# Onetism/LightFieldMicroscopy_PC-bzip2

Hardware: NVIDIA B200
Metric: compress+decompress round-trip GB/s (raw uint16) (higher is better)
Workload: dtype u16

## Files before the change

lightfieldmicroscopy_pc-bzip2_b200/csrc/bz_bwt.cu:

```cuda
#include "lfm_radix.cuh"
#include <cstdlib>

namespace lfm {

enum { S_SA0 = 0, S_SA1, S_ISA, S_G0, S_G1, S_R0, S_R1, S_V0, S_V1, S_U0, S_U1, S_COUNT };

extern __shared__ __align__(16) uint8_t bwt_smem[];

template <int NT>
__global__ void __launch_bounds__(NT, NT == 1024 ? 1 : 4)
k_bwt(const uint8_t* __restrict__ txt_all, uint32_t cap, EncJob* __restrict__ jobs, uint32_t njobs,
      uint8_t* __restrict__ bwt_all, uint32_t* __restrict__ scratch_all, int text_in_smem, int prefix_forced)
{
	constexpr int BWT_NT = NT;
	uint32_t* wcnt = reinterpret_cast<uint32_t*>(bwt_smem);
	uint32_t* base = reinterpret_cast<uint32_t*>(bwt_smem + (NT / 32) * BWT_WS * 4);
	uint32_t* run  = base + 256;
	uint32_t* red  = run + 256;
	uint32_t* misc = red + 64;
	uint8_t*  stext = reinterpret_cast<uint8_t*>(misc + 16);

	uint32_t* scr = scratch_all + (size_t)blockIdx.x * S_COUNT * cap;
	const uint32_t tid = threadIdx.x;

	for (uint32_t job = blockIdx.x; job < njobs; job += gridDim.x) {
		const uint32_t n = jobs[job].n;
		const uint8_t* gtext = txt_all + (size_t)job * cap;
		uint8_t* bwt = bwt_all + (size_t)job * cap;
		if (n == 0) { if (tid == 0) { jobs[job].orig_ptr = 0; jobs[job].periodic = 0; } continue; }

		const uint8_t* text;
		if (text_in_smem) {
			for (uint32_t i = tid * 4; i < n; i += BWT_NT * 4) {
				uint32_t wv = *reinterpret_cast<const uint32_t*>(gtext + i);
				*reinterpret_cast<uint32_t*>(stext + i) = wv;
			}
			__syncthreads();
			if (tid < 8) stext[n + tid] = stext[tid % n];
			text = stext;
		} else {
			text = gtext;
		}
		__syncthreads();
		digit_starts<NT>(n, base, wcnt, red, [&](uint32_t e) { return (uint32_t)text[e]; });
		if (tid < 256) {
			const uint32_t c = (tid == 255 ? n : base[tid + 1]) - base[tid];
			const uint32_t bal = __ballot_sync(0xffffffffu, c != 0);
			if ((tid & 31) == 0) jobs[job].in_use[tid >> 5] = bal;
		}

		const int prefix = prefix_forced ? prefix_forced : (n <= 49152u ? 6 : 8);
		uint32_t* src = nullptr; uint32_t* dst = scr + (size_t)S_SA0 * cap;
		for (int p = prefix - 1; p >= 0; p--) {
			if (tid < 256) run[tid] = base[tid];
			__syncthreads();
			const uint32_t* s = src; uint32_t* d = dst;
			radix_scatter<BWT_R, uint32_t, NT>(n, run, wcnt,
				[&](uint32_t e) { return s ? s[e] : e; },
				[&](uint32_t idx) { return (uint32_t)text[idx + p]; },
				[&](uint32_t pos, uint32_t idx) { d[pos] = idx; });
			src = dst;
			dst = (dst == scr + (size_t)S_SA0 * cap) ? scr + (size_t)S_SA1 * cap : scr + (size_t)S_SA0 * cap;
		}
		uint32_t* sa = src;
		uint32_t* isa = scr + (size_t)S_ISA * cap;

		uint32_t* G[2] = { scr + (size_t)S_G0 * cap, scr + (size_t)S_G1 * cap };
		uint32_t* Rk[2] = { scr + (size_t)S_R0 * cap, scr + (size_t)S_R1 * cap };
		uint32_t* V[2] = { scr + (size_t)S_V0 * cap, scr + (size_t)S_V1 * cap };
		uint32_t* U[2] = { scr + (size_t)S_U0 * cap, scr + (size_t)S_U1 * cap };
		const uint64_t pmask = prefix >= 8 ? ~0ull : ((1ull << (8 * prefix)) - 1ull);
		uint32_t m = split_groups<NT>(n, red,
			[&](uint32_t j) -> uint64_t {
				const uint32_t idx = sa[j], sh = (idx & 3u) * 8u;
				const uint32_t* tw = reinterpret_cast<const uint32_t*>(text + (idx & ~3u));
				const uint32_t w0 = tw[0], w1 = tw[1], w2 = tw[2];
				return (((uint64_t)__funnelshift_r(w1, w2, sh) << 32) | __funnelshift_r(w0, w1, sh)) & pmask;
			},
			[&](uint32_t j) { return j; },
			[&](uint32_t j, uint32_t head, bool un, uint32_t slot) {
				uint32_t sfx = sa[j];
				isa[sfx] = head;
				if (un) { G[0][slot] = head; V[0][slot] = sfx; U[0][slot] = j; }
			});

		const int npass = n <= (1u << 8) ? 1 : n <= (1u << 16) ? 2 : 3;
		int cur = 0, ucur = 0;
		uint64_t h = (uint64_t)prefix;
		while (m > 0 && h < n) {
			uint32_t hh = (uint32_t)h;
			for (uint32_t e = tid; e < m; e += BWT_NT) {
				uint32_t i = V[cur][e] + hh; if (i >= n) i -= n;
				Rk[cur][e] = isa[i];
			}
			__syncthreads();
			for (int key = 0; key < 2; key++) {
				for (int ps = 0; ps < npass; ps++) {
					const uint32_t* kg = G[cur]; const uint32_t* kr = Rk[cur]; const uint32_t* kv = V[cur];
					uint32_t* og = G[cur ^ 1]; uint32_t* orr = Rk[cur ^ 1]; uint32_t* ov = V[cur ^ 1];
					const int sh = ps * 8;
					digit_starts<NT>(m, run, wcnt, red, [&](uint32_t e) { return ((key ? kg[e] : kr[e]) >> sh) & 255u; });
					radix_scatter<4, Trip, NT>(m, run, wcnt,
						[&](uint32_t e) { Trip t; t.g = kg[e]; t.r = kr[e]; t.v = kv[e]; return t; },
						[&](const Trip& t) { return ((key ? t.g : t.r) >> sh) & 255u; },
						[&](uint32_t pos, const Trip& t) { og[pos] = t.g; orr[pos] = t.r; ov[pos] = t.v; });
					cur ^= 1;
				}
			}
			{
				const uint32_t* kg = G[cur]; const uint32_t* kr = Rk[cur]; const uint32_t* kv = V[cur];
				const uint32_t* up = U[ucur];
				uint32_t* ng = G[cur ^ 1]; uint32_t* nv = V[cur ^ 1]; uint32_t* nu = U[ucur ^ 1];
				const uint32_t mm = m;
				m = split_groups<NT>(mm, red,
					[&](uint32_t s) -> uint64_t { return ((uint64_t)kg[s] << 32) | kr[s]; },
					[&](uint32_t s) { return up[s]; },
					[&](uint32_t s, uint32_t head, bool un, uint32_t slot) {
						uint32_t sfx = kv[s], pos = up[s];
						sa[pos] = sfx;
						isa[sfx] = head;
						if (un) { ng[slot] = head; nv[slot] = sfx; nu[slot] = pos; }
					});
				cur ^= 1; ucur ^= 1;
			}
			__syncthreads();
			h <<= 1;
		}

		for (uint32_t j = tid * 4; j < n; j += BWT_NT * 4) {
			const uint4 q = *reinterpret_cast<const uint4*>(sa + j);
			const uint32_t sv[4] = { q.x, q.y, q.z, q.w };
			uint32_t wv = 0;
			#pragma unroll
			for (int k = 0; k < 4; k++) if (j + k < n) {
				const uint32_t s = sv[k];
				wv |= (uint32_t)text[s ? s - 1 : n - 1] << (8 * k);
				if (s == 0 && m == 0) jobs[job].orig_ptr = j + k;
			}
			*reinterpret_cast<uint32_t*>(bwt + j) = wv;
		}
		if (m > 0) {
			if (tid == 0) misc[1] = 0;
			__syncthreads();
			uint32_t g0 = isa[0], c = 0;
			for (uint32_t e = tid; e < m; e += BWT_NT) c += (G[cur][e] == g0);
			if (c) atomicAdd(&misc[1], c);
			__syncthreads();
			if (tid == 0) jobs[job].orig_ptr = g0 + misc[1] - 1;
		}
		if (tid == 0) jobs[job].periodic = m > 0;
		__syncthreads();
	}
}

static size_t bwt_smem_bytes_nt(uint32_t cap, int text_in_smem, int nt)
{
	size_t fixed = (size_t)(nt / 32) * BWT_WS * 4 + (256 + 256 + 64 + 16) * 4;
	return fixed + (text_in_smem ? (size_t)cap + 16 : 0);
}
size_t bwt_smem_bytes(uint32_t cap, int text_in_smem) { return bwt_smem_bytes_nt(cap, text_in_smem, BWT_NT); }
size_t bwt_scratch_elems_per_cta(uint32_t cap) { return (size_t)S_COUNT * cap; }
int bwt_ctas_per_sm(uint32_t cap, int text_in_smem)
{
	static const int forced = getenv("LFM_B200_BWT_NT") ? atoi(getenv("LFM_B200_BWT_NT")) : 0;
	if (forced == 1024) return 1;
	return (text_in_smem && bwt_smem_bytes_nt(cap, 1, 256) + 1024 <= (size_t)227 * 1024 / 4) ? 4 : 1;
}

void launch_bwt(const uint8_t* txt, uint32_t cap, EncJob* jobs, uint32_t njobs, uint8_t* bwt, uint32_t* scratch,
                int grid, int text_in_smem, cudaStream_t st)
{
	static const int prefix = getenv("LFM_B200_BWT_PREFIX") ? std::min(8, std::max(2, atoi(getenv("LFM_B200_BWT_PREFIX")))) : 0;
	if (bwt_ctas_per_sm(cap, text_in_smem) == 4) {
		const size_t smem = bwt_smem_bytes_nt(cap, text_in_smem, 256);
		cudaFuncSetAttribute(k_bwt<256>, cudaFuncAttributeMaxDynamicSharedMemorySize, (int)smem);
		k_bwt<256><<<grid, 256, smem, st>>>(txt, cap, jobs, njobs, bwt, scratch, text_in_smem, prefix);
		return;
	}
	const size_t smem = bwt_smem_bytes_nt(cap, text_in_smem, 1024);
	cudaFuncSetAttribute(k_bwt<1024>, cudaFuncAttributeMaxDynamicSharedMemorySize, (int)smem);
	k_bwt<1024><<<grid, 1024, smem, st>>>(txt, cap, jobs, njobs, bwt, scratch, text_in_smem, prefix);
}

}
```

lightfieldmicroscopy_pc-bzip2_b200/csrc/lfm_radix.cuh:

```cuda
#pragma once
#include "lfm_device.cuh"

namespace lfm {

constexpr int BWT_NT = 1024;
constexpr int BWT_R  = 12;
constexpr int BWT_NW = BWT_NT / 32;
constexpr int BWT_WS = 257;
constexpr int SPLIT_R = 4;
#define LFM_WC(w, d) wcnt[(w) * BWT_WS + (d)]

struct Trip { uint32_t g, r, v; };

template <int R, class P, int NT = BWT_NT, class LoadFn, class DigitFn, class StoreFn>
__device__ __forceinline__ void radix_scatter(uint32_t m, uint32_t* run, uint32_t* wcnt,
                                              LoadFn load, DigitFn digit, StoreFn store)
{
	const uint32_t lane = lane_id(), w = warp_id();
	const uint32_t lt = (1u << lane) - 1u;
	constexpr uint32_t TILE = NT * R;
	uint32_t* myc = wcnt + w * BWT_WS;
	__syncthreads();
	for (uint32_t i = lane; i < BWT_WS; i += 32) myc[i] = 0;
	__syncwarp();
	for (uint32_t t0 = 0; t0 < m; t0 += TILE) {
		P pay[R]; uint32_t dl[R];
		const uint32_t eb = t0 + w * (32 * R) + lane;
		#pragma unroll
		for (int r = 0; r < R; r++) if (eb + r * 32 < m) pay[r] = load(eb + r * 32);
		#pragma unroll
		for (int r = 0; r < R; r++) dl[r] = (eb + r * 32 < m) ? digit(pay[r]) : 256u;
		constexpr int RH = R > 8 ? R / 2 : R;
		#pragma unroll
		for (int r0 = 0; r0 < R; r0 += RH) {
			uint32_t peers[RH], old[RH];
			#pragma unroll
			for (int r = 0; r < RH; r++) peers[r] = __match_any_sync(0xffffffffu, dl[r0 + r]);
			#pragma unroll
			for (int r = 0; r < RH; r++) {
				old[r] = 0;
				if ((peers[r] & lt) == 0) old[r] = atomicAdd(&myc[dl[r0 + r]], (uint32_t)__popc(peers[r]));
				__syncwarp();
			}
			#pragma unroll
			for (int r = 0; r < RH; r++) {
				const uint32_t o = __shfl_sync(0xffffffffu, old[r], __ffs(peers[r]) - 1);
				dl[r0 + r] = (dl[r0 + r] << 16) | (o + __popc(peers[r] & lt));
			}
		}
		__syncthreads();
		if constexpr (NT == 256) {
			const uint32_t d = threadIdx.x;
			uint32_t* col = wcnt + d;
			uint32_t c[8];
			#pragma unroll
			for (int i = 0; i < 8; i++) c[i] = col[i * BWT_WS];
			uint32_t acc = run[d];
			#pragma unroll
			for (int i = 0; i < 8; i++) { col[i * BWT_WS] = acc; acc += c[i]; }
			run[d] = acc;
		} else {
			static_assert(NT == 1024, "scan layouts exist for 1024 and 256 threads");
			const uint32_t d = threadIdx.x >> 2, part = threadIdx.x & 3u;
			uint32_t* col = wcnt + (part * 8) * BWT_WS + d;
			uint32_t c[8], tot = 0;
			#pragma unroll
			for (int i = 0; i < 8; i++) { c[i] = col[i * BWT_WS]; tot += c[i]; }
			uint32_t incl = tot;
			uint32_t t1 = __shfl_up_sync(0xffffffffu, incl, 1); if (part >= 1) incl += t1;
			uint32_t t2 = __shfl_up_sync(0xffffffffu, incl, 2); if (part >= 2) incl += t2;
			uint32_t acc = run[d] + incl - tot;
			#pragma unroll
			for (int i = 0; i < 8; i++) { col[i * BWT_WS] = acc; acc += c[i]; }
			__syncwarp();
			if (part == 3) run[d] = acc;
		}
		__syncthreads();
		#pragma unroll
		for (int r = 0; r < R; r++) if (eb + r * 32 < m) store(myc[dl[r] >> 16] + (dl[r] & 0xffffu), pay[r]);
		__syncwarp();
		for (uint32_t i = lane; i < BWT_WS; i += 32) myc[i] = 0;
		__syncwarp();
	}
	__syncthreads();
}

template <bool SCAN, int NT = BWT_NT, class DigitOfIndex>
__device__ __forceinline__ void digit_hist(uint32_t m, uint32_t* run, uint32_t* wcnt, uint32_t* red, DigitOfIndex dig)
{
	const uint32_t lane = lane_id(), w = warp_id();
	const uint32_t lt = (1u << lane) - 1u;
	uint32_t* myc = wcnt + w * BWT_WS;
	constexpr int U = 4;
	__syncthreads();
	for (uint32_t i = lane; i < BWT_WS; i += 32) myc[i] = 0;
	__syncwarp();
	for (uint32_t e0 = w * (32 * U); e0 < m; e0 += NT * U) {
		uint32_t d[U], peers[U];
		#pragma unroll
		for (int u = 0; u < U; u++) { const uint32_t e = e0 + u * 32 + lane; d[u] = e < m ? dig(e) : 256u; }
		#pragma unroll
		for (int u = 0; u < U; u++) peers[u] = __match_any_sync(0xffffffffu, d[u]);
		#pragma unroll
		for (int u = 0; u < U; u++) if ((peers[u] & lt) == 0) atomicAdd(&myc[d[u]], (uint32_t)__popc(peers[u]));
	}
	__syncthreads();
	if (threadIdx.x < 256) {
		uint32_t s = 0;
		#pragma unroll 8
		for (int ww = 0; ww < NT / 32; ww++) s += LFM_WC(ww, threadIdx.x);
		run[threadIdx.x] = s;
	}
	__syncthreads();
	if (SCAN) scan256_excl<NT>(run, red);
}
template <int NT = BWT_NT, class DigitOfIndex>
__device__ __forceinline__ void digit_starts(uint32_t m, uint32_t* run, uint32_t* wcnt, uint32_t* red, DigitOfIndex dig)
{
	digit_hist<true, NT>(m, run, wcnt, red, dig);
}

template <int NT = BWT_NT, class KeyFn, class PosFn, class EmitFn>
__device__ __forceinline__ uint32_t split_groups(uint32_t cnt, uint32_t* red, KeyFn key_of, PosFn pos_of, EmitFn emit)
{
	uint32_t carry_head = 0, carry_cnt = 0;
	for (uint32_t t0 = 0; t0 < cnt; t0 += NT * SPLIT_R) {
		uint32_t i0 = t0 + threadIdx.x * SPLIT_R;
		bool hd[SPLIT_R + 1]; uint32_t gh[SPLIT_R];
		{
			uint64_t ky[SPLIT_R + 2];
			#pragma unroll
			for (int r = 0; r < SPLIT_R + 2; r++) { const uint32_t j = i0 + r; ky[r] = (j >= 1 && j <= cnt) ? key_of(j - 1) : 0; }
			#pragma unroll
			for (int r = 0; r <= SPLIT_R; r++) { const uint32_t j = i0 + r; hd[r] = (j == 0 || j >= cnt) ? true : (ky[r] != ky[r + 1]); }
		}
		uint32_t local = 0;
		#pragma unroll
		for (int r = 0; r < SPLIT_R; r++) { if (i0 + r < cnt && hd[r]) local = pos_of(i0 + r); gh[r] = local; }
		uint32_t incl = block_scan_max<NT>(local, red);
		uint32_t tile_max = red[NT / 32 - 1];
		uint32_t before = __shfl_up_sync(0xffffffffu, incl, 1);
		if (lane_id() == 0) before = warp_id() ? red[warp_id() - 1] : 0;
		before = max(before, carry_head);
		uint32_t c = 0; bool un[SPLIT_R];
		#pragma unroll
		for (int r = 0; r < SPLIT_R; r++) {
			gh[r] = max(gh[r], before);
			un[r] = (i0 + r < cnt) && !(hd[r] && hd[r + 1]);
			c += un[r];
		}
		uint32_t tot; uint32_t inc = block_scan_add<NT>(c, red, &tot);
		uint32_t o = carry_cnt + inc - c;
		#pragma unroll
		for (int r = 0; r < SPLIT_R; r++) if (i0 + r < cnt) { emit(i0 + r, gh[r], un[r], o); o += un[r]; }
		carry_cnt += tot;
		carry_head = max(carry_head, tile_max);
	}
	__syncthreads();
	return carry_cnt;
}

}
```

Measured before the change: 2.399.

## Sort BWT prefix by dense byte-pair ranks with segmented counting passes

When the block has at most 2048 distinct byte pairs, the kernel builds a bitmap of the pairs present, gives each pair a dense 16-bit rank, and sorts the initial prefix by these ranks. This halves the number of LSD radix passes. Each pass is a segmented counting sort that packs two 16-bit counters into each shared word and carries the rank in the upper bits of the stored value. It adds an extra pass over the text, a rank array written into the ISA scratch space, and a larger shared-memory footprint. Optional clock64 phase instrumentation is included behind a compile flag.

Result: slower. 2.262, median of 6 (-5.7%).

```diff
diff --git a/lightfieldmicroscopy_pc-bzip2_b200/csrc/bz_bwt.cu b/lightfieldmicroscopy_pc-bzip2_b200/csrc/bz_bwt.cu
--- a/lightfieldmicroscopy_pc-bzip2_b200/csrc/bz_bwt.cu
+++ b/lightfieldmicroscopy_pc-bzip2_b200/csrc/bz_bwt.cu
@@ -2,6 +2,19 @@
 #include <cstdlib>
 
 namespace lfm {
+
+#ifdef LFM_BWT_PHASE_CLOCKS
+__device__ unsigned long long bwt_phase_cycles[5];
+#define BWT_PHASE(k) do { if (tid == 0) { const long long t1 = clock64(); atomicAdd(&bwt_phase_cycles[k], (unsigned long long)(t1 - t_ph)); t_ph = t1; } } while (0)
+#else
+#define BWT_PHASE(k) do { } while (0)
+#endif
+
+__host__ __device__ constexpr size_t bwt_cnt_bytes(int nt, bool pairs)
+{
+	return (size_t)(nt / 32) * BWT_WS * 4 + 512 * 4 > (pairs ? (size_t)(nt / 32) * SEG_NB * 2 : 0)
+	     ? (size_t)(nt / 32) * BWT_WS * 4 + 512 * 4 : (size_t)(nt / 32) * SEG_NB * 2;
+}
 
 enum { S_SA0 = 0, S_SA1, S_ISA, S_G0, S_G1, S_R0, S_R1, S_V0, S_V1, S_U0, S_U1, S_COUNT };
 
@@ -10,13 +23,13 @@
 template <int NT>
 __global__ void __launch_bounds__(NT, NT == 1024 ? 1 : 4)
 k_bwt(const uint8_t* __restrict__ txt_all, uint32_t cap, EncJob* __restrict__ jobs, uint32_t njobs,
-      uint8_t* __restrict__ bwt_all, uint32_t* __restrict__ scratch_all, int text_in_smem, int prefix_forced)
+      uint8_t* __restrict__ bwt_all, uint32_t* __restrict__ scratch_all, int text_in_smem, int prefix_forced, int pair_smem)
 {
 	constexpr int BWT_NT = NT;
 	uint32_t* wcnt = reinterpret_cast<uint32_t*>(bwt_smem);
 	uint32_t* base = reinterpret_cast<uint32_t*>(bwt_smem + (NT / 32) * BWT_WS * 4);
 	uint32_t* run  = base + 256;
-	uint32_t* red  = run + 256;
+	uint32_t* red  = reinterpret_cast<uint32_t*>(bwt_smem + bwt_cnt_bytes(NT, pair_smem));
 	uint32_t* misc = red + 64;
 	uint8_t*  stext = reinterpret_cast<uint8_t*>(misc + 16);
 
@@ -28,6 +41,9 @@
 		const uint8_t* gtext = txt_all + (size_t)job * cap;
 		uint8_t* bwt = bwt_all + (size_t)job * cap;
 		if (n == 0) { if (tid == 0) { jobs[job].orig_ptr = 0; jobs[job].periodic = 0; } continue; }
+#ifdef LFM_BWT_PHASE_CLOCKS
+		long long t_ph = clock64();
+#endif
 
 		const uint8_t* text;
 		if (text_in_smem) {
@@ -42,26 +58,72 @@
 			text = gtext;
 		}
 		__syncthreads();
-		digit_starts<NT>(n, base, wcnt, red, [&](uint32_t e) { return (uint32_t)text[e]; });
-		if (tid < 256) {
-			const uint32_t c = (tid == 255 ? n : base[tid + 1]) - base[tid];
-			const uint32_t bal = __ballot_sync(0xffffffffu, c != 0);
-			if ((tid & 31) == 0) jobs[job].in_use[tid >> 5] = bal;
-		}
-
 		const int prefix = prefix_forced ? prefix_forced : (n <= 49152u ? 6 : 8);
+		uint16_t* rho = reinterpret_cast<uint16_t*>(scr + (size_t)S_ISA * cap);
+		bool pairs = false;
+		uint32_t D = 0;
+		if (NT == 256 && pair_smem && (prefix & 1) == 0) {
+			uint32_t* bm = wcnt;
+			uint16_t* wpre = reinterpret_cast<uint16_t*>(wcnt + 2048);
+			for (uint32_t i = tid; i < 2048 / 4; i += BWT_NT) reinterpret_cast<uint4*>(bm)[i] = make_uint4(0, 0, 0, 0);
+			__syncthreads();
+			for (uint32_t i = tid; i < n; i += BWT_NT) {
+				const uint32_t key = (uint32_t)text[i] << 8 | text[i + 1], bit = 1u << (key & 31);
+				if (!(bm[key >> 5] & bit)) atomicOr(&bm[key >> 5], bit);
+			}
+			__syncthreads();
+			uint32_t c[8], cs = 0;
+			#pragma unroll
+			for (int k = 0; k < 8; k++) { c[k] = __popc(bm[8 * tid + k]); cs += c[k]; }
+			uint32_t pre = block_scan_add<NT>(cs, red, &D) - cs;
+			#pragma unroll
+			for (int k = 0; k < 8; k++) { wpre[8 * tid + k] = (uint16_t)pre; pre += c[k]; }
+			pairs = D <= (uint32_t)SEG_NB;
+			if (pairs) {
+				const uint32_t bal = __ballot_sync(0xffffffffu, cs != 0);
+				if ((tid & 31) == 0) jobs[job].in_use[tid >> 5] = bal;
+				__syncthreads();
+				for (uint32_t i = tid; i < n + 4; i += BWT_NT) {
+					const uint32_t key = (uint32_t)text[i] << 8 | text[i + 1];
+					rho[i] = (uint16_t)(wpre[key >> 5] + __popc(bm[key >> 5] & ((1u << (key & 31)) - 1u)));
+				}
+			}
+			__syncthreads();
+		}
+		if (!pairs) {
+			digit_starts<NT>(n, base, wcnt, red, [&](uint32_t e) { return (uint32_t)text[e]; });
+			if (tid < 256) {
+				const uint32_t c = (tid == 255 ? n : base[tid + 1]) - base[tid];
+				const uint32_t bal = __ballot_sync(0xffffffffu, c != 0);
+				if ((tid & 31) == 0) jobs[job].in_use[tid >> 5] = bal;
+			}
+		}
+		BWT_PHASE(0);
+
 		uint32_t* src = nullptr; uint32_t* dst = scr + (size_t)S_SA0 * cap;
-		for (int p = prefix - 1; p >= 0; p--) {
-			if (tid < 256) run[tid] = base[tid];
-			__syncthreads();
+		const int npass = pairs ? prefix / 2 : prefix;
+		const uint32_t nbits = D > 1 ? 32 - __clz(D - 1) : 0;
+		for (int p = npass - 1; p >= 0; p--) {
 			const uint32_t* s = src; uint32_t* d = dst;
-			radix_scatter<BWT_R, uint32_t, NT>(n, run, wcnt,
-				[&](uint32_t e) { return s ? s[e] : e; },
-				[&](uint32_t idx) { return (uint32_t)text[idx + p]; },
-				[&](uint32_t pos, uint32_t idx) { d[pos] = idx; });
+			if (pairs) {
+				const uint32_t off = 2 * p;
+				if constexpr (NT == 256)
+					seg_counting_pass<NT>(n, nbits, wcnt, red,
+						[&](uint32_t e) { return s ? s[e] : (uint32_t)rho[e + off] << 16 | e; },
+						[&](uint32_t v) { const uint32_t idx = v & 0xffffu; return p ? (uint32_t)rho[idx + off - 2] << 16 | idx : idx; },
+						[&](uint32_t pos, uint32_t v) { d[pos] = v; });
+			} else {
+				if (tid < 256) run[tid] = base[tid];
+				__syncthreads();
+				radix_scatter<BWT_R, uint32_t, NT>(n, run, wcnt,
+					[&](uint32_t e) { return s ? s[e] : e; },
+					[&](uint32_t idx) { return (uint32_t)text[idx + p]; },
+					[&](uint32_t pos, uint32_t idx) { d[pos] = idx; });
+			}
 			src = dst;
 			dst = (dst == scr + (size_t)S_SA0 * cap) ? scr + (size_t)S_SA1 * cap : scr + (size_t)S_SA0 * cap;
 		}
+		BWT_PHASE(1);
 		uint32_t* sa = src;
 		uint32_t* isa = scr + (size_t)S_ISA * cap;
 
@@ -83,8 +145,9 @@
 				isa[sfx] = head;
 				if (un) { G[0][slot] = head; V[0][slot] = sfx; U[0][slot] = j; }
 			});
-
-		const int npass = n <= (1u << 8) ? 1 : n <= (1u << 16) ? 2 : 3;
+		BWT_PHASE(2);
+
+		const int nrpass = n <= (1u << 8) ? 1 : n <= (1u << 16) ? 2 : 3;
 		int cur = 0, ucur = 0;
 		uint64_t h = (uint64_t)prefix;
 		while (m > 0 && h < n) {
@@ -95,7 +158,7 @@
 			}
 			__syncthreads();
 			for (int key = 0; key < 2; key++) {
-				for (int ps = 0; ps < npass; ps++) {
+				for (int ps = 0; ps < nrpass; ps++) {
 					const uint32_t* kg = G[cur]; const uint32_t* kr = Rk[cur]; const uint32_t* kv = V[cur];
 					uint32_t* og = G[cur ^ 1]; uint32_t* orr = Rk[cur ^ 1]; uint32_t* ov = V[cur ^ 1];
 					const int sh = ps * 8;
@@ -126,6 +189,7 @@
 			__syncthreads();
 			h <<= 1;
 		}
+		BWT_PHASE(3);
 
 		for (uint32_t j = tid * 4; j < n; j += BWT_NT * 4) {
 			const uint4 q = *reinterpret_cast<const uint4*>(sa + j);
@@ -150,12 +214,13 @@
 		}
 		if (tid == 0) jobs[job].periodic = m > 0;
 		__syncthreads();
+		BWT_PHASE(4);
 	}
 }
 
-static size_t bwt_smem_bytes_nt(uint32_t cap, int text_in_smem, int nt)
-{
-	size_t fixed = (size_t)(nt / 32) * BWT_WS * 4 + (256 + 256 + 64 + 16) * 4;
+static size_t bwt_smem_bytes_nt(uint32_t cap, int text_in_smem, int nt, bool pairs = false)
+{
+	size_t fixed = bwt_cnt_bytes(nt, pairs) + (64 + 16) * 4;
 	return fixed + (text_in_smem ? (size_t)cap + 16 : 0);
 }
 size_t bwt_smem_bytes(uint32_t cap, int text_in_smem) { return bwt_smem_bytes_nt(cap, text_in_smem, BWT_NT); }
@@ -171,15 +236,17 @@
                 int grid, int text_in_smem, cudaStream_t st)
 {
 	static const int prefix = getenv("LFM_B200_BWT_PREFIX") ? std::min(8, std::max(2, atoi(getenv("LFM_B200_BWT_PREFIX")))) : 0;
+	static const bool pairs_on = !(getenv("LFM_B200_BWT_PAIRS") && atoi(getenv("LFM_B200_BWT_PAIRS")) == 0);
 	if (bwt_ctas_per_sm(cap, text_in_smem) == 4) {
-		const size_t smem = bwt_smem_bytes_nt(cap, text_in_smem, 256);
+		const bool pairs = pairs_on && bwt_smem_bytes_nt(cap, 1, 256, true) + 1024 <= (size_t)227 * 1024 / 4;
+		const size_t smem = bwt_smem_bytes_nt(cap, text_in_smem, 256, pairs);
 		cudaFuncSetAttribute(k_bwt<256>, cudaFuncAttributeMaxDynamicSharedMemorySize, (int)smem);
-		k_bwt<256><<<grid, 256, smem, st>>>(txt, cap, jobs, njobs, bwt, scratch, text_in_smem, prefix);
+		k_bwt<256><<<grid, 256, smem, st>>>(txt, cap, jobs, njobs, bwt, scratch, text_in_smem, prefix, (int)pairs);
 		return;
 	}
 	const size_t smem = bwt_smem_bytes_nt(cap, text_in_smem, 1024);
 	cudaFuncSetAttribute(k_bwt<1024>, cudaFuncAttributeMaxDynamicSharedMemorySize, (int)smem);
-	k_bwt<1024><<<grid, 1024, smem, st>>>(txt, cap, jobs, njobs, bwt, scratch, text_in_smem, prefix);
-}
-
-}
+	k_bwt<1024><<<grid, 1024, smem, st>>>(txt, cap, jobs, njobs, bwt, scratch, text_in_smem, prefix, 0);
+}
+
+}
diff --git a/lightfieldmicroscopy_pc-bzip2_b200/csrc/lfm_radix.cuh b/lightfieldmicroscopy_pc-bzip2_b200/csrc/lfm_radix.cuh
--- a/lightfieldmicroscopy_pc-bzip2_b200/csrc/lfm_radix.cuh
+++ b/lightfieldmicroscopy_pc-bzip2_b200/csrc/lfm_radix.cuh
@@ -120,6 +120,105 @@
 	digit_hist<true, NT>(m, run, wcnt, red, dig);
 }
 
+constexpr int SEG_NB = 2048;
+#ifndef SEG_HIST_MATCH
+#define SEG_HIST_MATCH 1
+#endif
+#ifndef SEG_BALLOT
+#define SEG_BALLOT 0
+#endif
+#ifndef SEG_NBITS_ALL
+#define SEG_NBITS_ALL 1
+#endif
+__device__ __forceinline__ uint32_t seg_peers(uint32_t d, bool valid, uint32_t nbits)
+{
+#if SEG_BALLOT
+	uint32_t p = __ballot_sync(0xffffffffu, valid);
+	#pragma unroll
+	for (int b = 0; b < 11; b++)
+		if (SEG_NBITS_ALL || b < nbits) { const uint32_t q = __ballot_sync(0xffffffffu, (d >> b) & 1u); p &= ((d >> b) & 1u) ? q : ~q; }
+	return p;
+#else
+	return __match_any_sync(0xffffffffu, valid ? d : 0xffffu);
+#endif
+}
+template <int NT, class ElemFn, class NextFn, class StoreFn>
+__device__ __forceinline__ void seg_counting_pass(uint32_t m, uint32_t nbits, uint32_t* cnt, uint32_t* red, ElemFn elem, NextFn next, StoreFn store)
+{
+	static_assert(NT * 8 == SEG_NB, "the scan gives every thread 8 digits");
+	constexpr uint32_t NW = NT / 32, ROW = SEG_NB / 2, U = 4, NONE = 0xffffu;
+	const uint32_t lane = lane_id(), w = warp_id(), lt = (1u << lane) - 1u;
+	uint32_t* myc = cnt + w * ROW;
+	const uint32_t seg = (m + NW * 32 - 1) / (NW * 32) * 32;
+	const uint32_t lo = min(w * seg, m), hi = min(lo + seg, m);
+	for (uint32_t i = lane; i < ROW / 4; i += 32) reinterpret_cast<uint4*>(myc)[i] = make_uint4(0, 0, 0, 0);
+	__syncwarp();
+	for (uint32_t e0 = lo; e0 < hi; e0 += 32 * U) {
+		uint32_t d[U];
+		#pragma unroll
+		for (int u = 0; u < U; u++) { const uint32_t e = e0 + u * 32 + lane; d[u] = e < hi ? elem(e) >> 16 : NONE; }
+#if SEG_HIST_MATCH
+		uint32_t peers[U];
+		#pragma unroll
+		for (int u = 0; u < U; u++) peers[u] = seg_peers(d[u], d[u] != NONE, nbits);
+		#pragma unroll
+		for (int u = 0; u < U; u++)
+			if (d[u] != NONE && (peers[u] & lt) == 0) atomicAdd(&myc[d[u] >> 1], (uint32_t)__popc(peers[u]) << (16 * (d[u] & 1)));
+#else
+		#pragma unroll
+		for (int u = 0; u < U; u++) if (d[u] != NONE) atomicAdd(&myc[d[u] >> 1], 1u << (16 * (d[u] & 1)));
+#endif
+	}
+	__syncthreads();
+	{
+		const uint32_t t = threadIdx.x;
+		uint4 tot = make_uint4(0, 0, 0, 0);
+		#pragma unroll
+		for (uint32_t i = 0; i < NW; i++) {
+			const uint4 c = reinterpret_cast<const uint4*>(cnt + i * ROW)[t];
+			tot.x += c.x; tot.y += c.y; tot.z += c.z; tot.w += c.w;
+		}
+		const uint32_t tw[4] = { tot.x, tot.y, tot.z, tot.w };
+		uint32_t s = 0;
+		#pragma unroll
+		for (int k = 0; k < 4; k++) s += (tw[k] & 0xffffu) + (tw[k] >> 16);
+		uint32_t all, b = block_scan_add<NT>(s, red, &all) - s;
+		uint32_t st[4];
+		#pragma unroll
+		for (int k = 0; k < 4; k++) { const uint32_t b1 = b + (tw[k] & 0xffffu); st[k] = b | (b1 << 16); b = b1 + (tw[k] >> 16); }
+		uint4 acc = make_uint4(st[0], st[1], st[2], st[3]);
+		#pragma unroll
+		for (uint32_t i = 0; i < NW; i++) {
+			uint4* p = reinterpret_cast<uint4*>(cnt + i * ROW) + t;
+			const uint4 c = *p;
+			*p = acc;
+			acc.x += c.x; acc.y += c.y; acc.z += c.z; acc.w += c.w;
+		}
+	}
+	__syncthreads();
+	for (uint32_t e0 = lo; e0 < hi; e0 += 32 * U) {
+		uint32_t v[U], d[U], peers[U], old[U];
+		#pragma unroll
+		for (int u = 0; u < U; u++) { const uint32_t e = e0 + u * 32 + lane; v[u] = e < hi ? elem(e) : NONE << 16; d[u] = v[u] >> 16; }
+		#pragma unroll
+		for (int u = 0; u < U; u++) if (d[u] != NONE) v[u] = next(v[u]);
+		#pragma unroll
+		for (int u = 0; u < U; u++) peers[u] = seg_peers(d[u], d[u] != NONE, nbits);
+		#pragma unroll
+		for (int u = 0; u < U; u++) {
+			old[u] = 0;
+			if (d[u] != NONE && (peers[u] & lt) == 0) old[u] = atomicAdd(&myc[d[u] >> 1], (uint32_t)__popc(peers[u]) << (16 * (d[u] & 1)));
+			__syncwarp();
+		}
+		#pragma unroll
+		for (int u = 0; u < U; u++) {
+			const uint32_t o = __shfl_sync(0xffffffffu, old[u], __ffs(peers[u]) - 1);
+			if (d[u] != NONE) store(((o >> (16 * (d[u] & 1))) & 0xffffu) + __popc(peers[u] & lt), v[u]);
+		}
+	}
+	__syncthreads();
+}
+
 template <int NT = BWT_NT, class KeyFn, class PosFn, class EmitFn>
 __device__ __forceinline__ uint32_t split_groups(uint32_t cnt, uint32_t* red, KeyFn key_of, PosFn pos_of, EmitFn emit)
 {
```
